# wangjiarui153/AIGV-Assessor

Hardware: AMD Instinct MI355X
Metric: scored clips/sec (8-frame 448x448, InternVL2-8B stage-2 score eval) (higher is better)
Workload: dtype bf16

## Files before the change

### aigv-assessor_amd/csrc/slowfast.hip

```cpp
#include <hip/hip_runtime.h>

#include <algorithm>
#include <cmath>
#include <cstdarg>
#include <cstdio>
#include <cstring>
#include <map>
#include <string>
#include <vector>

#include "../../include/aigv_amd.h"
#include "common.h"
#include "kernels.h"

namespace {

struct ConvArgs {
  const bf16_t* in;
  const bf16_t* w;
  const float* bias;
  const bf16_t* res;
  bf16_t* out;
  int ld_in, Cin, Ti, Hi, Wi;
  int kt, kh, kw, st, sh, sw, pt, ph, pw;
  int To, Ho, Wo, Cout, CoutPad, Kp;
  int ld_res, ld_out, c_off, relu;
  long rows;
  float* part;
  int k_slices;
};

template <int BN>
__global__ __launch_bounds__(256) void conv3d_mfma_kernel(ConvArgs p) {
  constexpr int BM = 128, BK = 64, NT = BN / 16, WJ = (BN + 31) / 32;
  __shared__ __attribute__((aligned(16))) bf16_t sA[BM * BK];
  __shared__ __attribute__((aligned(16))) bf16_t sW[BN * BK];
  const int tid = threadIdx.x, lane = tid & 63, wave = tid >> 6;
  const long m0 = (long)blockIdx.x * BM;
  const int n0 = blockIdx.y * BN;
  const int kspan = p.Kp / p.k_slices, kb = blockIdx.z * kspan;
  const int kc = tid & 7;
  const int r0 = tid >> 3;
  long base[4];
  int t0[4], y0[4], x0[4];
  bool rv[4];
#pragma unroll
  for (int j = 0; j < 4; ++j) {
    const long m = m0 + r0 + 32 * j;
    rv[j] = m < p.rows;
    const long mm = rv[j] ? m : 0;
    const int x = (int)(mm % p.Wo);
    const long r1 = mm / p.Wo;
    const int y = (int)(r1 % p.Ho);
    const long r2 = r1 / p.Ho;
    const int t = (int)(r2 % p.To);
    const long b = r2 / p.To;
    t0[j] = t * p.st - p.pt;
    y0[j] = y * p.sh - p.ph;
    x0[j] = x * p.sw - p.pw;
    base[j] = b * p.Ti * p.Hi * p.Wi;
  }
  int c = kb + kc * 8, dx = 0, dy = 0, dt = 0;
  auto normalise = [&]() {
    while (c >= p.Cin) {
      c -= p.Cin;
      if (++dx == p.kw) {
        dx = 0;
        if (++dy == p.kh) { dy = 0; ++dt; }
      }
    }
  };
  normalise();
  auto gather = [&](int j) -> u16x8 {
    u16x8 z = {0, 0, 0, 0, 0, 0, 0, 0};
    if (!rv[j] || dt >= p.kt) return z;
    const int tt = t0[j] + dt, yy = y0[j] + dy, xx = x0[j] + dx;
    if ((unsigned)tt >= (unsigned)p.Ti || (unsigned)yy >= (unsigned)p.Hi || (unsigned)xx >= (unsigned)p.Wi) return z;
    return *(const u16x8*)(p.in + (base[j] + ((long)tt * p.Hi + yy) * p.Wi + xx) * p.ld_in + c);
  };
  bool wv[WJ];
  const bf16_t* wsrc[WJ];
#pragma unroll
  for (int j = 0; j < WJ; ++j) {
    const int wrow = r0 + 32 * j;
    wv[j] = wrow < BN && (n0 + wrow) < p.CoutPad;
    wsrc[j] = p.w + (size_t)(n0 + (wv[j] ? wrow : 0)) * p.Kp + kb + kc * 8;
  }
  f32x4 acc[2][NT];
#pragma unroll
  for (int i = 0; i < 2; ++i)
#pragma unroll
    for (int n = 0; n < NT; ++n) acc[i][n] = f32x4{0.f, 0.f, 0.f, 0.f};

  const u16x8 zero = {0, 0, 0, 0, 0, 0, 0, 0};
  u16x8 ra[4], rw[WJ];
#pragma unroll
  for (int j = 0; j < 4; ++j) ra[j] = gather(j);
#pragma unroll
  for (int j = 0; j < WJ; ++j) rw[j] = wv[j] ? *(const u16x8*)wsrc[j] : zero;
  const int slot = (kc ^ (r0 & 7)) * 8;
  for (int k0 = 0; k0 < kspan; k0 += BK) {
    __syncthreads();
#pragma unroll
    for (int j = 0; j < 4; ++j) *(u16x8*)&sA[(r0 + 32 * j) * BK + slot] = ra[j];
#pragma unroll
    for (int j = 0; j < WJ; ++j)
      if (r0 + 32 * j < BN) *(u16x8*)&sW[(r0 + 32 * j) * BK + slot] = rw[j];
    __syncthreads();
    if (k0 + BK < kspan) {
      c += BK;
      normalise();
#pragma unroll
      for (int j = 0; j < 4; ++j) ra[j] = gather(j);
#pragma unroll
      for (int j = 0; j < WJ; ++j) rw[j] = wv[j] ? *(const u16x8*)(wsrc[j] + k0 + BK) : zero;
    }
#pragma unroll
    for (int h = 0; h < 2; ++h) {
      const int rs = ((h * 4 + (lane >> 4)) ^ (lane & 7)) * 8;
      bf16x8 a[2], w[NT];
#pragma unroll
      for (int i = 0; i < 2; ++i) a[i] = *(const bf16x8*)&sA[(wave * 32 + i * 16 + (lane & 15)) * BK + rs];
#pragma unroll
      for (int n = 0; n < NT; ++n) w[n] = *(const bf16x8*)&sW[(n * 16 + (lane & 15)) * BK + rs];
#pragma unroll
      for (int i = 0; i < 2; ++i)
#pragma unroll
        for (int n = 0; n < NT; ++n) acc[i][n] = __builtin_amdgcn_mfma_f32_16x16x32_bf16(w[n], a[i], acc[i][n], 0, 0, 0);
    }
  }
#pragma unroll
  for (int i = 0; i < 2; ++i) {
    const long m = m0 + wave * 32 + i * 16 + (lane & 15);
    if (m >= p.rows) continue;
#pragma unroll
    for (int n = 0; n < NT; ++n) {
      const int ch = n0 + n * 16 + (lane >> 4) * 4;
      if (ch >= p.Cout) continue;
      if (p.k_slices > 1) {
        *(f32x4*)(p.part + ((size_t)blockIdx.z * p.rows + m) * p.Cout + ch) = acc[i][n];
        continue;
      }
      float v[4];
#pragma unroll
      for (int e = 0; e < 4; ++e) v[e] = acc[i][n][e] + p.bias[ch + e];
      if (p.res) {
        const u16x4 r = *(const u16x4*)(p.res + m * p.ld_res + ch);
#pragma unroll
        for (int e = 0; e < 4; ++e) v[e] += bf2f(r[e]);
      }
      u16x4 o;
#pragma unroll
      for (int e = 0; e < 4; ++e) o[e] = f2bf(p.relu ? fmaxf(v[e], 0.f) : v[e]);
      *(u16x4*)(p.out + m * p.ld_out + p.c_off + ch) = o;
    }
  }
}

__global__ __launch_bounds__(256) void conv_finalize_kernel(ConvArgs p) {
  const long i = (long)blockIdx.x * 256 + threadIdx.x;
  const int cq = p.Cout >> 2;
  if (i >= p.rows * cq) return;
  const long m = i / cq;
  const int ch = (int)(i - m * cq) * 4;
  f32x4 v = *(const f32x4*)(p.part + (size_t)m * p.Cout + ch);
  for (int z = 1; z < p.k_slices; ++z) v += *(const f32x4*)(p.part + ((size_t)z * p.rows + m) * p.Cout + ch);
#pragma unroll
  for (int e = 0; e < 4; ++e) v[e] += p.bias[ch + e];
  if (p.res) {
    const u16x4 r = *(const u16x4*)(p.res + m * p.ld_res + ch);
#pragma unroll
    for (int e = 0; e < 4; ++e) v[e] += bf2f(r[e]);
  }
  u16x4 o;
#pragma unroll
  for (int e = 0; e < 4; ++e) o[e] = f2bf(p.relu ? fmaxf(v[e], 0.f) : v[e]);
  *(u16x4*)(p.out + m * p.ld_out + p.c_off + ch) = o;
}

struct FrameIdx { int v[64]; };
__global__ __launch_bounds__(256) void sf_repack_kernel(const bf16_t* __restrict__ frames, int T, int Ts, long hw, bf16_t* __restrict__ fast,
                                                        bf16_t* __restrict__ slow, FrameIdx idx, long total) {
  const long i = (long)blockIdx.x * 256 + threadIdx.x;
  if (i >= total) return;
  const long px = i % hw;
  const long f = i / hw;
  const int tt = (int)(f % (T + Ts));
  const long b = f / (T + Ts);
  const int src_t = tt < T ? tt : idx.v[tt - T];
  const bf16_t* s = frames + ((b * T + src_t) * 3) * hw + px;
  u16x4 o = {s[0], s[hw], s[2 * hw], 0};
  bf16_t* d = tt < T ? fast + ((b * T + tt) * hw + px) * 4 : slow + ((b * Ts + (tt - T)) * hw + px) * 4;
  *(u16x4*)d = o;
}

__global__ __launch_bounds__(256) void sf_maxpool_kernel(const bf16_t* __restrict__ in, int C, int Hi, int Wi, int Ho, int Wo,
                                                         bf16_t* __restrict__ out, int ld_out, long total) {
  const long i = (long)blockIdx.x * 256 + threadIdx.x;
  if (i >= total) return;
  const int cv = C >> 3;
  const int c8 = (int)(i % cv);
  const long px = i / cv;
  const int x = (int)(px % Wo);
  const long r = px / Wo;
  const int y = (int)(r % Ho);
  const long f = r / Ho;
  float m[8];
#pragma unroll
  for (int e = 0; e < 8; ++e) m[e] = -INFINITY;
  for (int dy = 0; dy < 3; ++dy) {
    const int yy = 2 * y - 1 + dy;
    if ((unsigned)yy >= (unsigned)Hi) continue;
    for (int dx = 0; dx < 3; ++dx) {
      const int xx = 2 * x - 1 + dx;
      if ((unsigned)xx >= (unsigned)Wi) continue;
      const u16x8 v = *(const u16x8*)(in + ((f * Hi + yy) * Wi + xx) * C + c8 * 8);
#pragma unroll
      for (int e = 0; e < 8; ++e) m[e] = fmaxf(m[e], bf2f(v[e]));
    }
  }
  u16x8 o;
#pragma unroll
  for (int e = 0; e < 8; ++e) o[e] = f2bf(m[e]);
  *(u16x8*)(out + px * ld_out + c8 * 8) = o;
}

struct PoolW { float t[32], y[32], x[32]; };
__global__ __launch_bounds__(256) void sf_pool_kernel(const bf16_t* __restrict__ in, int T, int H, int W, int C, PoolW w,
                                                      bf16_t* __restrict__ out, int ld_out, int c_off) {
  __shared__ float red[64][4][8];
  const int chunk = threadIdx.x & 3, slice = threadIdx.x >> 2;
  const int c8 = blockIdx.x * 4 + chunk;
  const int b = blockIdx.y;
  float acc[8] = {0.f, 0.f, 0.f, 0.f, 0.f, 0.f, 0.f, 0.f};
  if (c8 * 8 < C) {
    const bf16_t* s = in + (long)b * T * H * W * C + c8 * 8;
    const int n = T * H * W;
    for (int i = slice; i < n; i += 64) {
      const int x = i % W, r = i / W, y = r % H, t = r / H;
      const float wt = w.t[t] * w.y[y] * w.x[x];
      const u16x8 v = *(const u16x8*)(s + (long)i * C);
#pragma unroll
      for (int e = 0; e < 8; ++e) acc[e] += wt * bf2f(v[e]);
    }
  }
#pragma unroll
  for (int e = 0; e < 8; ++e) red[slice][chunk][e] = acc[e];
  __syncthreads();
  if (threadIdx.x < 32 && (blockIdx.x * 4 + (threadIdx.x >> 3)) * 8 < C) {
    const int ch = threadIdx.x >> 3, e = threadIdx.x & 7;
    float v = 0.f;
    for (int q = 0; q < 64; ++q) v += red[q][ch][e];
    out[(long)b * ld_out + c_off + (blockIdx.x * 4 + ch) * 8 + e] = f2bf(v);
  }
}

constexpr long SPLITK_MAX_ROWS = 8192;

int conv_k_slices(long rows, int CoutPad, int Kp) {
  if (rows > SPLITK_MAX_ROWS || Kp < 1024) return 1;
  const int bn = CoutPad >= 64 ? 64 : CoutPad >= 32 ? 32 : 16;
  const long tiles = ((rows + 127) / 128) * ((CoutPad + bn - 1) / bn);
  if (tiles >= 64) return 1;
  const int steps = Kp / 64;
  for (int S : {8, 6, 4, 3, 2})
    if (steps % S == 0 && steps / S >= 4 && tiles * S <= 512) return S;
  return 1;
}

hipError_t launch_conv(const ConvArgs& a_in, hipStream_t s, int S = 1, float* ws = nullptr, size_t ws_floats = 0) {
  ConvArgs a = a_in;
  if (a.rows <= 0) return hipSuccess;
  if (a.Cin % 8 || a.ld_in % 8 || a.Cout % 4 || a.ld_out % 4 || a.c_off % 4 || a.Kp % 64 || a.CoutPad % 16 || (a.res && a.ld_res % 4) ||
      a.Kp < a.kt * a.kh * a.kw * a.Cin)
    return hipErrorInvalidValue;
  if (!ws || S < 1 || (a.Kp / 64) % S || (size_t)S * a.rows * a.Cout > ws_floats) S = 1;
  a.k_slices = S;
  a.part = S > 1 ? ws : nullptr;
  const unsigned gx = (unsigned)((a.rows + 127) / 128);
  if (a.CoutPad >= 64) hipLaunchKernelGGL(conv3d_mfma_kernel<64>, dim3(gx, (a.CoutPad + 63) / 64, S), dim3(256), 0, s, a);
  else if (a.CoutPad >= 32) hipLaunchKernelGGL(conv3d_mfma_kernel<32>, dim3(gx, (a.CoutPad + 31) / 32, S), dim3(256), 0, s, a);
  else hipLaunchKernelGGL(conv3d_mfma_kernel<16>, dim3(gx, 1, S), dim3(256), 0, s, a);
  if (S > 1) {
    const long total = a.rows * (a.Cout / 4);
    hipLaunchKernelGGL(conv_finalize_kernel, dim3((unsigned)((total + 255) / 256)), dim3(256), 0, s, a);
  }
  return hipGetLastError();
}

inline uint16_t bf16_host(float f) {
  uint32_t u;
  memcpy(&u, &f, 4);
  if ((u & 0x7fffffffu) > 0x7f800000u) return (uint16_t)((u >> 16) | 0x40);
  u += 0x7fffu + ((u >> 16) & 1u);
  return (uint16_t)(u >> 16);
}
inline float bf16_to_float_host(uint16_t h) {
  uint32_t u = (uint32_t)h << 16;
  float f;
  memcpy(&f, &u, 4);
  return f;
}

struct HostTensor {
  std::vector<float> v;
  std::vector<int64_t> shape;
};

enum OpKind { OP_REPACK, OP_CONV, OP_MAXPOOL, OP_POOL };
struct Op {
  OpKind kind;
  ConvArgs a{};
  int in_buf = -1, out_buf = -1, res_buf = -1;
  size_t w_off = 0, b_off = 0;
  long rows_per_clip = 0;
  int k_slices = 1;
  int C = 0, T = 0, Hi = 0, Wi = 0, Ho = 0, Wo = 0, ld_out = 0, c_off = 0;
  PoolW pw{};
};

int sf_fail(int code, const char* fmt, ...) {
  char buf[768];
  va_list ap;
  va_start(ap, fmt);
  vsnprintf(buf, sizeof buf, fmt, ap);
  va_end(ap);
  aigv_set_error(buf);
  return code;
}

}

struct aigv_slowfast {
  int device = 0, Bcap = 0, T = 0, Ts = 0, H = 0, W = 0;
  bool finalized = false;
  std::map<std::string, HostTensor> host;
  std::vector<Op> ops;
  std::vector<size_t> buf_elems;
  std::vector<bf16_t*> bufs;
  bf16_t* d_w = nullptr;
  float* d_b = nullptr;
  float* d_part = nullptr;
  size_t part_floats = 0;
  FrameIdx slow_idx{};
  double flops_per_clip = 0;
};

namespace {

enum { B_IN0 = 0, B_IN1, B_STEM0, B_STEM1, B_X00, B_X01, B_X10, B_X11, B_A0, B_A1, B_B0, B_B1, B_S0, B_S1, B_COUNT };

struct Builder {
  aigv_slowfast* sf;
  std::vector<uint16_t> w;
  std::vector<float> b;
  std::string missing;

  const HostTensor* get(const std::string& name) {
    auto it = sf->host.find(name);
    if (it == sf->host.end()) {
      if (missing.size() < 400) missing += (missing.empty() ? "" : ", ") + name;
      return nullptr;
    }
    return &it->second;
  }
  void need(int buf, size_t elems) {
    if (sf->buf_elems[buf] < elems) sf->buf_elems[buf] = elems;
  }
  bool conv(const std::string& conv_name, const std::string& norm_name, int in_buf, int ld_in, int cin_eff, int Ti, int Hi, int Wi, int kt, int kh,
            int kw, int st, int sh, int sw, int pt, int ph, int pw, int cout, int out_buf, int ld_out, int c_off, int res_buf, int ld_res, bool relu,
            int* To_, int* Ho_, int* Wo_, bool stem_pairs = false) {
    const HostTensor* W = get(conv_name + ".weight");
    const HostTensor* g = get(norm_name + ".weight");
    const HostTensor* be = get(norm_name + ".bias");
    const HostTensor* mu = get(norm_name + ".running_mean");
    const HostTensor* var = get(norm_name + ".running_var");
    const int To = (Ti + 2 * pt - kt) / st + 1, Ho = (Hi + 2 * ph - kh) / sh + 1, Wo = (Wi + 2 * pw - kw) / sw + 1;
    *To_ = To; *Ho_ = Ho; *Wo_ = Wo;
    if (!W || !g || !be || !mu || !var) return false;
    const int cin_real = W->shape.size() == 5 ? (int)W->shape[1] : -1;
    if (W->shape.size() != 5 || W->shape[0] != cout || (stem_pairs ? cin_real != 3 : cin_real != cin_eff) || W->shape[2] != kt || W->shape[3] != kh || W->shape[4] != kw ||
        (int)g->v.size() != cout || (int)be->v.size() != cout || (int)mu->v.size() != cout || (int)var->v.size() != cout) {
      if (missing.size() < 400) missing += (missing.empty() ? "" : ", ") + conv_name + " (bad shape)";
      return false;
    }
    const int taps = kt * kh * kw;
    const int kw_k = stem_pairs ? 4 : kw, taps_k = kt * kh * kw_k;
    const int K = taps_k * cin_eff, Kp = (K + 63) / 64 * 64, coutPad = (cout + 15) / 16 * 16;
    Op op;
    op.kind = OP_CONV;
    op.w_off = w.size();
    op.b_off = b.size();
    w.resize(w.size() + (size_t)coutPad * Kp, 0);
    b.resize(b.size() + cout, 0.f);
    for (int co = 0; co < cout; ++co) {
      const float scale = g->v[co] / std::sqrt(var->v[co] + 1e-5f);
      b[op.b_off + co] = be->v[co] - mu->v[co] * scale;
      uint16_t* dst = &w[op.w_off + (size_t)co * Kp];
      for (int ci = 0; ci < cin_real; ++ci)
        for (int tap = 0; tap < taps; ++tap) {
          int k = tap * cin_eff + ci;
          if (stem_pairs) {
            const int q = tap % kw + 1;
            k = ((tap / kw) * 4 + (q >> 1)) * 8 + (q & 1) * 4 + ci;
          }
          dst[k] = bf16_host(W->v[((size_t)co * cin_real + ci) * taps + tap] * scale);
        }
    }
    ConvArgs& a = op.a;
    a.ld_in = ld_in; a.Cin = cin_eff; a.Ti = Ti; a.Hi = Hi; a.Wi = stem_pairs ? Wi / 2 : Wi;
    a.kt = kt; a.kh = kh; a.kw = kw_k; a.st = st; a.sh = sh; a.sw = stem_pairs ? 1 : sw; a.pt = pt; a.ph = ph; a.pw = stem_pairs ? 2 : pw;
    a.To = To; a.Ho = Ho; a.Wo = Wo; a.Cout = cout; a.CoutPad = coutPad; a.Kp = Kp;
    a.ld_res = ld_res; a.ld_out = ld_out; a.c_off = c_off; a.relu = relu ? 1 : 0;
    op.in_buf = in_buf; op.out_buf = out_buf; op.res_buf = res_buf;
    op.rows_per_clip = (long)To * Ho * Wo;
    need(out_buf, (size_t)op.rows_per_clip * ld_out);
    sf->flops_per_clip += 2.0 * op.rows_per_clip * cout * (double)taps * cin_real;
    sf->ops.push_back(op);
    return true;
  }
};

void cover_weights(float* w, int n, int k) {
  for (int i = 0; i < n; ++i) {
    const int lo = i - k + 1 > 0 ? i - k + 1 : 0, hi = i < n - k ? i : n - k;
    w[i] = (float)(hi - lo + 1);
  }
}

}

extern "C" {

int aigv_slowfast_create(int device, int max_clips, int frames_per_clip, int height, int width, aigv_slowfast** out) {
  if (!out) return sf_fail(AIGV_ERR_ARG, "aigv_slowfast_create: null argument");
  *out = nullptr;
  int ndev = 0;
  if (hipGetDeviceCount(&ndev) != hipSuccess || ndev <= 0)
    return sf_fail(AIGV_ERR_HIP, "aigv_slowfast_create: no HIP device is visible (this library has no CPU fallback)");
  if (device < 0 || device >= ndev) return sf_fail(AIGV_ERR_ARG, "aigv_slowfast_create: device %d out of range (%d visible)", device, ndev);
  if (max_clips <= 0 || frames_per_clip < 8 || frames_per_clip > 32 || frames_per_clip % 4 || height < 224 || width < 224 || height % 32 ||
      width % 32 || height > 1024 || width > 1024)
    return sf_fail(AIGV_ERR_ARG, "aigv_slowfast_create: needs 8 <= T <= 32 with T %% 4 == 0 and 224 <= H, W <= 1024 multiples of 32 (got T=%d %dx%d)",
                   frames_per_clip, height, width);
  aigv_slowfast* sf = new (std::nothrow) aigv_slowfast();
  if (!sf) return sf_fail(AIGV_ERR_ALLOC, "out of host memory");
  sf->device = device; sf->Bcap = max_clips; sf->T = frames_per_clip; sf->Ts = frames_per_clip / 4; sf->H = height; sf->W = width;
  const int n = sf->Ts;
  const float step = n > 1 ? (float)(sf->T - 1) / (float)(n - 1) : 0.f;
  for (int i = 0; i < n; ++i) sf->slow_idx.v[i] = i < n / 2 ? (int)(0.f + step * i) : (int)((float)(sf->T - 1) - step * (float)(n - 1 - i));
  *out = sf;
  return 0;
}

void aigv_slowfast_destroy(aigv_slowfast* sf) {
  if (!sf) return;
  hipSetDevice(sf->device);
  hipDeviceSynchronize();
  for (bf16_t* p : sf->bufs) hipFree(p);
  hipFree(sf->d_w);
  hipFree(sf->d_b);
  hipFree(sf->d_part);
  delete sf;
}

int aigv_slowfast_load_weight(aigv_slowfast* sf, const char* name, const void* host_data, const int64_t* shape, int ndim, int dtype) {
  if (!sf || !name || !host_data || !shape || ndim <= 0 || ndim > 5) return sf_fail(AIGV_ERR_ARG, "aigv_slowfast_load_weight: bad argument");
  if (sf->finalized) return sf_fail(AIGV_ERR_STATE, "aigv_slowfast_load_weight(%s): already finalized", name);
  std::string key(name);
  for (const char* pre : {"slowfast_model.feature_extraction.", "feature_extraction.", "blocks."}) {
    const size_t n = strlen(pre);
    if (key.compare(0, n, pre) == 0) { key = key.substr(n); break; }
  }
  HostTensor t;
  size_t n = 1;
  for (int i = 0; i < ndim; ++i) {
    if (shape[i] <= 0) return sf_fail(AIGV_ERR_ARG, "aigv_slowfast_load_weight(%s): bad shape", name);
    n *= (size_t)shape[i];
    t.shape.push_back(shape[i]);
  }
  t.v.resize(n);
  if (dtype == AIGV_F32) memcpy(t.v.data(), host_data, n * 4);
  else if (dtype == AIGV_BF16) for (size_t i = 0; i < n; ++i) t.v[i] = bf16_to_float_host(((const uint16_t*)host_data)[i]);
  else return sf_fail(AIGV_ERR_ARG, "aigv_slowfast_load_weight(%s): dtype %d", name, dtype);
  sf->host[key] = std::move(t);
  return 0;
}

int aigv_slowfast_finalize(aigv_slowfast* sf) {
  if (!sf) return sf_fail(AIGV_ERR_ARG, "aigv_slowfast_finalize: null handle");
  if (sf->finalized) return 0;
  if (hipSetDevice(sf->device) != hipSuccess) return sf_fail(AIGV_ERR_HIP, "hipSetDevice failed");
  sf->ops.clear();
  sf->buf_elems.assign(B_COUNT, 0);
  sf->flops_per_clip = 0;
  Builder bd{sf, {}, {}, {}};
  const int T[2] = {sf->Ts, sf->T};
  const int IN[2] = {B_IN0, B_IN1}, STEM[2] = {B_STEM0, B_STEM1}, X[2][2] = {{B_X00, B_X01}, {B_X10, B_X11}}, A[2] = {B_A0, B_A1},
            Bq[2] = {B_B0, B_B1}, S[2] = {B_S0, B_S1};
  {
    Op op; op.kind = OP_REPACK;
    sf->ops.push_back(op);
    bd.need(B_IN0, (size_t)sf->Ts * sf->H * sf->W * 4);
    bd.need(B_IN1, (size_t)sf->T * sf->H * sf->W * 4);
  }
  bool ok = true;
  int h = 0, w = 0, to = 0;
  int ld[2] = {64 + 16, 8};
  for (int p = 0; p < 2; ++p) {
    const int kt = p ? 5 : 1, cout = p ? 8 : 64;
    const std::string pre = "0.multipathway_blocks." + std::to_string(p);
    ok &= bd.conv(pre + ".conv", pre + ".norm", IN[p], 8, 8, T[p], sf->H, sf->W, kt, 7, 7, 1, 2, 2, kt / 2, 3, 3, cout, STEM[p], cout, 0, -1, 0, true, &to, &h, &w, true);
    Op mp; mp.kind = OP_MAXPOOL;
    mp.in_buf = STEM[p]; mp.out_buf = X[p][0]; mp.C = cout; mp.T = T[p]; mp.Hi = h; mp.Wi = w;
    mp.Ho = (h + 2 - 3) / 2 + 1; mp.Wo = (w + 2 - 3) / 2 + 1; mp.ld_out = ld[p];
    bd.need(X[p][0], (size_t)T[p] * mp.Ho * mp.Wo * ld[p]);
    sf->ops.push_back(mp);
    if (p == 1) { h = mp.Ho; w = mp.Wo; }
  }
  int sp_h = h, sp_w = w;
  ok &= bd.conv("0.multipathway_fusion.conv_fast_to_slow", "0.multipathway_fusion.norm", X[1][0], 8, 8, T[1], sp_h, sp_w, 7, 1, 1, 4, 1, 1, 3, 0, 0, 16,
                X[0][0], ld[0], 64, -1, 0, true, &to, &h, &w);
  if (to != T[0]) return sf_fail(AIGV_ERR_ARG, "fast->slow fusion yields %d frames, slow pathway has %d", to, T[0]);
  int cur[2] = {0, 0};
  int cin[2] = {80, 8};
  static const int depths[4] = {3, 4, 6, 3};
  for (int s = 0; s < 4; ++s) {
    int out_h = sp_h, out_w = sp_w;
    for (int p = 0; p < 2; ++p) {
      const int inner = (p ? 8 : 64) << s, cout = inner * 4;
      const int fuse_ch = (s < 3 && p == 0) ? 2 * (32 << s) : 0;
      const int ld_out = cout + fuse_ch;
      const int kt_a = (p == 1 || s >= 2) ? 3 : 1;
      int bh = sp_h, bw = sp_w;
      for (int blk = 0; blk < depths[s]; ++blk) {
        const int stv = (blk == 0 && s > 0) ? 2 : 1;
        const std::string pre = std::to_string(s + 1) + ".multipathway_blocks." + std::to_string(p) + ".res_blocks." + std::to_string(blk) + ".";
        const int xin = X[p][cur[p]], xout = X[p][cur[p] ^ 1];
        const int c_in = blk == 0 ? cin[p] : cout, ld_in = blk == 0 ? ld[p] : ld_out;
        int t1, h1, w1, h2, w2;
        int res_buf = xin, res_ld = ld_in;
        if (blk == 0) {
          ok &= bd.conv(pre + "branch1_conv", pre + "branch1_norm", xin, ld_in, c_in, T[p], bh, bw, 1, 1, 1, 1, stv, stv, 0, 0, 0, cout, S[p], cout, 0, -1, 0,
                        false, &t1, &h1, &w1);
          res_buf = S[p]; res_ld = cout;
        }
        ok &= bd.conv(pre + "branch2.conv_a", pre + "branch2.norm_a", xin, ld_in, c_in, T[p], bh, bw, kt_a, 1, 1, 1, 1, 1, kt_a / 2, 0, 0, inner, A[p], inner, 0,
                      -1, 0, true, &t1, &h1, &w1);
        ok &= bd.conv(pre + "branch2.conv_b", pre + "branch2.norm_b", A[p], inner, inner, T[p], bh, bw, 1, 3, 3, 1, stv, stv, 0, 1, 1, inner, Bq[p], inner, 0, -1,
                      0, true, &t1, &h2, &w2);
        ok &= bd.conv(pre + "branch2.conv_c", pre + "branch2.norm_c", Bq[p], inner, inner, T[p], h2, w2, 1, 1, 1, 1, 1, 1, 0, 0, 0, cout, xout, ld_out, 0, res_buf,
                      res_ld, true, &t1, &h1, &w1);
        bh = h2; bw = w2;
        cur[p] ^= 1;
      }
      cin[p] = ld_out; ld[p] = ld_out;
      out_h = bh; out_w = bw;
    }
    sp_h = out_h; sp_w = out_w;
    if (s < 3) {
      const int cf = 32 << s, cs = 256 << s;
      const std::string pre = std::to_string(s + 1) + ".multipathway_fusion";
      ok &= bd.conv(pre + ".conv_fast_to_slow", pre + ".norm", X[1][cur[1]], cf, cf, T[1], sp_h, sp_w, 7, 1, 1, 4, 1, 1, 3, 0, 0, 2 * cf, X[0][cur[0]], ld[0], cs,
                    -1, 0, true, &to, &h, &w);
    }
  }
  if (!ok) return sf_fail(AIGV_ERR_STATE, "aigv_slowfast_finalize: missing or mis-shaped tensors: %s%s", bd.missing.c_str(), bd.missing.size() >= 400 ? " ..." : "");
  if (sp_h < 7 || sp_w < 7 || sp_h > 32 || sp_w > 32) return sf_fail(AIGV_ERR_ARG, "final map %dx%d outside the head pool's range", sp_h, sp_w);
  for (int p = 0; p < 2; ++p) {
    Op op; op.kind = OP_POOL;
    op.in_buf = X[p][cur[p]]; op.C = p ? 256 : 2048; op.T = T[p]; op.Hi = sp_h; op.Wi = sp_w; op.ld_out = 2304; op.c_off = p ? 2048 : 0;
    const int L = 4 * T[p], k = p ? 32 : 8;
    if (L < k) return sf_fail(AIGV_ERR_ARG, "too few frames for the head pool");
    float rep[128];
    cover_weights(rep, L, k);
    float ty[32], tx[32];
    cover_weights(ty, sp_h, 7);
    cover_weights(tx, sp_w, 7);
    const float nt = (float)(L - k + 1) * k, ny = (float)(sp_h - 6) * 7, nx = (float)(sp_w - 6) * 7;
    for (int t = 0; t < T[p]; ++t) op.pw.t[t] = (rep[4 * t] + rep[4 * t + 1] + rep[4 * t + 2] + rep[4 * t + 3]) / nt;
    for (int y = 0; y < sp_h; ++y) op.pw.y[y] = ty[y] / ny;
    for (int x = 0; x < sp_w; ++x) op.pw.x[x] = tx[x] / nx;
    sf->ops.push_back(op);
  }
  auto dmalloc = [&](void** p, size_t bytes) { return hipMalloc(p, bytes ? bytes : 16); };
  if (dmalloc((void**)&sf->d_w, bd.w.size() * 2) != hipSuccess || dmalloc((void**)&sf->d_b, bd.b.size() * 4) != hipSuccess)
    return sf_fail(AIGV_ERR_ALLOC, "aigv_slowfast_finalize: hipMalloc of %zu weight bytes failed", bd.w.size() * 2);
  if (hipMemcpy(sf->d_w, bd.w.data(), bd.w.size() * 2, hipMemcpyHostToDevice) != hipSuccess ||
      hipMemcpy(sf->d_b, bd.b.data(), bd.b.size() * 4, hipMemcpyHostToDevice) != hipSuccess)
    return sf_fail(AIGV_ERR_HIP, "aigv_slowfast_finalize: weight upload failed");
  sf->bufs.assign(B_COUNT, nullptr);
  for (int i = 0; i < B_COUNT; ++i) {
    const size_t bytes = sf->buf_elems[i] * (size_t)sf->Bcap * 2 + 64;
    if (hipMalloc((void**)&sf->bufs[i], bytes) != hipSuccess) return sf_fail(AIGV_ERR_ALLOC, "aigv_slowfast_finalize: hipMalloc(%zu) failed", bytes);
    if (hipMemset(sf->bufs[i], 0, bytes) != hipSuccess) return sf_fail(AIGV_ERR_HIP, "hipMemset failed");
  }
  size_t need = 0;
  for (Op& op : sf->ops) {
    if (op.kind != OP_CONV) continue;
    op.k_slices = conv_k_slices(op.rows_per_clip, op.a.CoutPad, op.a.Kp);
    if (op.k_slices > 1) need = std::max(need, (size_t)op.k_slices * op.rows_per_clip * sf->Bcap * op.a.Cout);
  }
  sf->part_floats = need;
  if (sf->part_floats && hipMalloc((void**)&sf->d_part, sf->part_floats * sizeof(float)) != hipSuccess)
    return sf_fail(AIGV_ERR_ALLOC, "aigv_slowfast_finalize: hipMalloc of the split-K workspace failed");
  sf->host.clear();
  sf->finalized = true;
  return 0;
}

double aigv_slowfast_flops_per_clip(const aigv_slowfast* sf) { return sf ? sf->flops_per_clip : 0.0; }

int aigv_slowfast_forward(aigv_slowfast* sf, const void* frames_nchw_bf16, int clips, void* feature_bf16, void* stream) {
  if (!sf || !frames_nchw_bf16 || !feature_bf16) return sf_fail(AIGV_ERR_ARG, "aigv_slowfast_forward: null argument");
  if (!sf->finalized) return sf_fail(AIGV_ERR_STATE, "aigv_slowfast_forward: call aigv_slowfast_finalize first");
  if (clips <= 0 || clips > sf->Bcap) return sf_fail(AIGV_ERR_ARG, "aigv_slowfast_forward: %d clips, capacity %d", clips, sf->Bcap);
  if (hipSetDevice(sf->device) != hipSuccess) return sf_fail(AIGV_ERR_HIP, "aigv_slowfast_forward: hipSetDevice(%d) failed", sf->device);
  hipStream_t s = (hipStream_t)stream;
  for (const Op& op : sf->ops) {
    hipError_t e = hipSuccess;
    switch (op.kind) {
      case OP_REPACK: {
        const long hw = (long)sf->H * sf->W, total = (long)clips * (sf->T + sf->Ts) * hw;
        hipLaunchKernelGGL(sf_repack_kernel, dim3((unsigned)((total + 255) / 256)), dim3(256), 0, s, (const bf16_t*)frames_nchw_bf16, sf->T, sf->Ts, hw,
                           sf->bufs[B_IN1], sf->bufs[B_IN0], sf->slow_idx, total);
        e = hipGetLastError();
        break;
      }
      case OP_CONV: {
        ConvArgs a = op.a;
        a.in = sf->bufs[op.in_buf]; a.out = sf->bufs[op.out_buf]; a.res = op.res_buf >= 0 ? sf->bufs[op.res_buf] : nullptr;
        a.w = sf->d_w + op.w_off; a.bias = sf->d_b + op.b_off;
        a.rows = op.rows_per_clip * clips;
        e = launch_conv(a, s, op.k_slices, sf->d_part, sf->part_floats);
        break;
      }
      case OP_MAXPOOL: {
        const long total = (long)clips * op.T * op.Ho * op.Wo * (op.C / 8);
        hipLaunchKernelGGL(sf_maxpool_kernel, dim3((unsigned)((total + 255) / 256)), dim3(256), 0, s, sf->bufs[op.in_buf], op.C, op.Hi, op.Wi, op.Ho, op.Wo,
                           sf->bufs[op.out_buf], op.ld_out, total);
        e = hipGetLastError();
        break;
      }
      case OP_POOL: {
        hipLaunchKernelGGL(sf_pool_kernel, dim3((op.C + 31) / 32, clips), dim3(256), 0, s, sf->bufs[op.in_buf], op.T, op.Hi, op.Wi, op.C, op.pw,
                           (bf16_t*)feature_bf16, op.ld_out, op.c_off);
        e = hipGetLastError();
        break;
      }
    }
    if (e != hipSuccess) return sf_fail(e == hipErrorInvalidValue ? AIGV_ERR_ARG : AIGV_ERR_HIP, "aigv_slowfast_forward: launch failed: %s", hipGetErrorString(e));
  }
  return 0;
}

int aigv_op_conv3d(const void* x, int ld_in, int Cin, int B, const int* dims, const void* w_packed, int Kp, const float* bias, int Cout, const void* res,
                   int ld_res, void* out, int ld_out, int c_off, int relu, void* stream) {
  if (!x || !dims || !w_packed || !bias || !out) return sf_fail(AIGV_ERR_ARG, "aigv_op_conv3d: null argument");
  ConvArgs a{};
  a.in = (const bf16_t*)x; a.ld_in = ld_in; a.Cin = Cin; a.Ti = dims[0]; a.Hi = dims[1]; a.Wi = dims[2];
  a.kt = dims[3]; a.kh = dims[4]; a.kw = dims[5]; a.st = dims[6]; a.sh = dims[7]; a.sw = dims[8]; a.pt = dims[9]; a.ph = dims[10]; a.pw = dims[11];
  if (a.kt <= 0 || a.kh <= 0 || a.kw <= 0 || a.st <= 0 || a.sh <= 0 || a.sw <= 0 || a.pt < 0 || a.ph < 0 || a.pw < 0 || B <= 0 || Cin <= 0 || Cout <= 0 ||
      ld_in < Cin || ld_out < c_off + Cout || (res && ld_res < Cout) || a.Ti + 2 * a.pt < a.kt || a.Hi + 2 * a.ph < a.kh || a.Wi + 2 * a.pw < a.kw)
    return sf_fail(AIGV_ERR_ARG, "aigv_op_conv3d: bad geometry");
  a.To = (a.Ti + 2 * a.pt - a.kt) / a.st + 1; a.Ho = (a.Hi + 2 * a.ph - a.kh) / a.sh + 1; a.Wo = (a.Wi + 2 * a.pw - a.kw) / a.sw + 1;
  a.w = (const bf16_t*)w_packed; a.Kp = Kp; a.bias = bias; a.Cout = Cout; a.CoutPad = (Cout + 15) / 16 * 16;
  a.res = (const bf16_t*)res; a.ld_res = ld_res; a.out = (bf16_t*)out; a.ld_out = ld_out; a.c_off = c_off; a.relu = relu;
  a.rows = (long)B * a.To * a.Ho * a.Wo;
  hipError_t e = launch_conv(a, (hipStream_t)stream);
  if (e != hipSuccess)
    return sf_fail(e == hipErrorInvalidValue ? AIGV_ERR_ARG : AIGV_ERR_HIP,
                   "aigv_op_conv3d (Cin=%d Cout=%d Kp=%d; needs Cin, ld_in %% 8 == 0, Cout, ld_out, c_off %% 4 == 0, Kp %% 64 == 0): %s", Cin, Cout, Kp, hipGetErrorString(e));
  return 0;
}

}
```

Baseline: 34.95.

## Add multi-stage LDS ring pipeline for SlowFast conv3d with direct global-to-LDS loads

Adds a new conv3d kernel that streams A and W tiles into a 2–4 stage shared-memory ring using direct global-to-LDS loads, with explicit vmcnt waits and a single barrier per k-step. The goal is to overlap the implicit-GEMM gathers with MFMA work instead of relying on register double-buffering. A heuristic picks the ring depth from grid size and the LDS budget, falling back to the old kernel otherwise. The epilogue is factored out and preloads bias and residual before the stores, the split-K finalize unrolls its slice loads, and waves_per_eu hints are added. Larger dynamic LDS can reduce occupancy, and the hand-written waitcnt logic is fragile.

```diff
diff --git a/aigv-assessor_amd/csrc/slowfast.hip b/aigv-assessor_amd/csrc/slowfast.hip
--- a/aigv-assessor_amd/csrc/slowfast.hip
+++ b/aigv-assessor_amd/csrc/slowfast.hip
@@ -31,7 +31,59 @@
 };
 
 template <int BN>
-__global__ __launch_bounds__(256) void conv3d_mfma_kernel(ConvArgs p) {
+__device__ __forceinline__ void conv_epilogue(const ConvArgs& p, const f32x4 (&acc)[2][BN / 16], long m0, int n0, int wave, int lane) {
+  constexpr int NT = BN / 16;
+  const long mr[2] = {m0 + wave * 32 + (lane & 15), m0 + wave * 32 + 16 + (lane & 15)};
+  const int ch0 = n0 + (lane >> 4) * 4;
+  if (p.k_slices > 1) {
+#pragma unroll
+    for (int i = 0; i < 2; ++i)
+#pragma unroll
+      for (int n = 0; n < NT; ++n)
+        if (mr[i] < p.rows && ch0 + n * 16 < p.Cout) *(f32x4*)(p.part + ((size_t)blockIdx.z * p.rows + mr[i]) * p.Cout + ch0 + n * 16) = acc[i][n];
+    return;
+  }
+  const long mc[2] = {mr[0] < p.rows ? mr[0] : p.rows - 1, mr[1] < p.rows ? mr[1] : p.rows - 1};
+  float bias[NT][4];
+  u16x4 res[2][NT];
+#pragma unroll
+  for (int n = 0; n < NT; ++n) {
+    const int cc = ch0 + n * 16 < p.Cout ? ch0 + n * 16 : p.Cout - 4;
+#pragma unroll
+    for (int e = 0; e < 4; ++e) bias[n][e] = p.bias[cc + e];
+  }
+  if (p.res) {
+#pragma unroll
+    for (int n = 0; n < NT; ++n) {
+      const int cc = ch0 + n * 16 < p.Cout ? ch0 + n * 16 : p.Cout - 4;
+#pragma unroll
+      for (int i = 0; i < 2; ++i) res[i][n] = *(const u16x4*)(p.res + mc[i] * p.ld_res + cc);
+    }
+  }
+#pragma unroll
+  for (int i = 0; i < 2; ++i) {
+    if (mr[i] >= p.rows) continue;
+#pragma unroll
+    for (int n = 0; n < NT; ++n) {
+      const int ch = ch0 + n * 16;
+      if (ch >= p.Cout) continue;
+      float v[4];
+#pragma unroll
+      for (int e = 0; e < 4; ++e) v[e] = acc[i][n][e] + bias[n][e];
+      if (p.res) {
+#pragma unroll
+        for (int e = 0; e < 4; ++e) v[e] += bf2f(res[i][n][e]);
+      }
+      u16x4 o;
+#pragma unroll
+      for (int e = 0; e < 4; ++e) o[e] = f2bf(p.relu ? fmaxf(v[e], 0.f) : v[e]);
+      *(u16x4*)(p.out + mr[i] * p.ld_out + p.c_off + ch) = o;
+    }
+  }
+}
+
+template <int BN>
+__global__ __launch_bounds__(256) __attribute__((amdgpu_waves_per_eu(4))) void conv3d_mfma_kernel(ConvArgs p) {
   constexpr int BM = 128, BK = 64, NT = BN / 16, WJ = (BN + 31) / 32;
   __shared__ __attribute__((aligned(16))) bf16_t sA[BM * BK];
   __shared__ __attribute__((aligned(16))) bf16_t sW[BN * BK];
@@ -129,33 +181,112 @@
         for (int n = 0; n < NT; ++n) acc[i][n] = __builtin_amdgcn_mfma_f32_16x16x32_bf16(w[n], a[i], acc[i][n], 0, 0, 0);
     }
   }
-#pragma unroll
-  for (int i = 0; i < 2; ++i) {
-    const long m = m0 + wave * 32 + i * 16 + (lane & 15);
-    if (m >= p.rows) continue;
-#pragma unroll
-    for (int n = 0; n < NT; ++n) {
-      const int ch = n0 + n * 16 + (lane >> 4) * 4;
-      if (ch >= p.Cout) continue;
-      if (p.k_slices > 1) {
-        *(f32x4*)(p.part + ((size_t)blockIdx.z * p.rows + m) * p.Cout + ch) = acc[i][n];
-        continue;
+  conv_epilogue<BN>(p, acc, m0, n0, wave, lane);
+}
+
+__device__ __attribute__((aligned(16))) bf16_t g_sf_zero[8];
+
+template <int N>
+__device__ __forceinline__ void wait_vmcnt() { asm volatile("s_waitcnt vmcnt(%0)" ::"n"(N) : "memory"); }
+
+template <int BN, int NS>
+__global__ __launch_bounds__(256) __attribute__((amdgpu_waves_per_eu(4))) void conv3d_ring_kernel(ConvArgs p) {
+  constexpr int BM = 128, BK = 64, NT = BN / 16, WR = BN < 32 ? 32 : BN, WI = WR / 32;
+  constexpr int A_BYTES = BM * BK * 2, STAGE = A_BYTES + WR * BK * 2, NI = 4 + WI;
+  static_assert(NS >= 2 && (NS - 2) * NI <= 63, "vmcnt range");
+  extern __shared__ __attribute__((aligned(16))) char smem[];
+  const int tid = threadIdx.x, lane = tid & 63, wave = tid >> 6;
+  const long m0 = (long)blockIdx.x * BM;
+  const int n0 = blockIdx.y * BN;
+  const int kspan = p.Kp / p.k_slices, kb = blockIdx.z * kspan, steps = kspan / BK;
+  const int r0 = wave * 8 + (lane >> 3);
+  const int kc = (lane & 7) ^ ((lane >> 3) & 7);
+  const bf16_t* const zero = g_sf_zero;
+  long base[4];
+  int t0[4], y0[4], x0[4];
+  bool rv[4];
+#pragma unroll
+  for (int j = 0; j < 4; ++j) {
+    const long m = m0 + r0 + 32 * j;
+    rv[j] = m < p.rows;
+    const long mm = rv[j] ? m : 0;
+    const int x = (int)(mm % p.Wo);
+    const long r1 = mm / p.Wo;
+    const int y = (int)(r1 % p.Ho);
+    const long r2 = r1 / p.Ho;
+    const int t = (int)(r2 % p.To);
+    const long b = r2 / p.To;
+    t0[j] = t * p.st - p.pt;
+    y0[j] = y * p.sh - p.ph;
+    x0[j] = x * p.sw - p.pw;
+    base[j] = b * p.Ti * p.Hi * p.Wi;
+  }
+  int c = kb + kc * 8, dx = 0, dy = 0, dt = 0;
+  auto normalise = [&]() {
+    while (c >= p.Cin) {
+      c -= p.Cin;
+      if (++dx == p.kw) {
+        dx = 0;
+        if (++dy == p.kh) { dy = 0; ++dt; }
       }
-      float v[4];
-#pragma unroll
-      for (int e = 0; e < 4; ++e) v[e] = acc[i][n][e] + p.bias[ch + e];
-      if (p.res) {
-        const u16x4 r = *(const u16x4*)(p.res + m * p.ld_res + ch);
-#pragma unroll
-        for (int e = 0; e < 4; ++e) v[e] += bf2f(r[e]);
-      }
-      u16x4 o;
-#pragma unroll
-      for (int e = 0; e < 4; ++e) o[e] = f2bf(p.relu ? fmaxf(v[e], 0.f) : v[e]);
-      *(u16x4*)(p.out + m * p.ld_out + p.c_off + ch) = o;
-    }
-  }
-}
+    }
+  };
+  normalise();
+  auto gather = [&](int j) -> const bf16_t* {
+    if (!rv[j] || dt >= p.kt) return zero;
+    const int tt = t0[j] + dt, yy = y0[j] + dy, xx = x0[j] + dx;
+    if ((unsigned)tt >= (unsigned)p.Ti || (unsigned)yy >= (unsigned)p.Hi || (unsigned)xx >= (unsigned)p.Wi) return zero;
+    return p.in + (base[j] + ((long)tt * p.Hi + yy) * p.Wi + xx) * p.ld_in + c;
+  };
+  const bf16_t* wsrc[WI];
+#pragma unroll
+  for (int j = 0; j < WI; ++j) {
+    const int wrow = r0 + 32 * j;
+    wsrc[j] = (wrow < BN && n0 + wrow < p.CoutPad) ? p.w + (size_t)(n0 + wrow) * p.Kp + kb + kc * 8 : nullptr;
+  }
+  const unsigned lds0 = __builtin_amdgcn_readfirstlane((unsigned)(size_t)(LDS_AS char*)smem + wave * 1024);
+  auto issue = [&](int k) {
+    if (k >= steps) return;
+    const unsigned dst = lds0 + (unsigned)(k % NS) * STAGE;
+#pragma unroll
+    for (int j = 0; j < 4; ++j) glds16_asm(gather(j), dst + j * 4096);
+#pragma unroll
+    for (int j = 0; j < WI; ++j) glds16_asm(wsrc[j] ? wsrc[j] + k * BK : zero, dst + A_BYTES + j * 4096);
+    c += BK;
+    normalise();
+  };
+  f32x4 acc[2][NT];
+#pragma unroll
+  for (int i = 0; i < 2; ++i)
+#pragma unroll
+    for (int n = 0; n < NT; ++n) acc[i][n] = f32x4{0.f, 0.f, 0.f, 0.f};
+#pragma unroll
+  for (int k = 0; k < NS - 1; ++k) issue(k);
+  for (int k = 0; k < steps; ++k) {
+    if (k + NS - 2 < steps) wait_vmcnt<(NS - 2) * NI>();
+    else wait_vmcnt<0>();
+    asm volatile("s_barrier" ::: "memory");
+    issue(k + NS - 1);
+    const bf16_t* sA = (const bf16_t*)(smem + (k % NS) * STAGE);
+    const bf16_t* sW = (const bf16_t*)(smem + (k % NS) * STAGE + A_BYTES);
+#pragma unroll
+    for (int h = 0; h < 2; ++h) {
+      const int rs = ((h * 4 + (lane >> 4)) ^ (lane & 7)) * 8;
+      bf16x8 a[2], w[NT];
+#pragma unroll
+      for (int i = 0; i < 2; ++i) a[i] = *(const bf16x8*)&sA[(wave * 32 + i * 16 + (lane & 15)) * BK + rs];
+#pragma unroll
+      for (int n = 0; n < NT; ++n) w[n] = *(const bf16x8*)&sW[(n * 16 + (lane & 15)) * BK + rs];
+#pragma unroll
+      for (int i = 0; i < 2; ++i)
+#pragma unroll
+        for (int n = 0; n < NT; ++n) acc[i][n] = __builtin_amdgcn_mfma_f32_16x16x32_bf16(w[n], a[i], acc[i][n], 0, 0, 0);
+    }
+  }
+  conv_epilogue<BN>(p, acc, m0, n0, wave, lane);
+}
+
+constexpr int SPLITK_MAX_SLICES = 8;
 
 __global__ __launch_bounds__(256) void conv_finalize_kernel(ConvArgs p) {
   const long i = (long)blockIdx.x * 256 + threadIdx.x;
@@ -163,8 +294,14 @@
   if (i >= p.rows * cq) return;
   const long m = i / cq;
   const int ch = (int)(i - m * cq) * 4;
-  f32x4 v = *(const f32x4*)(p.part + (size_t)m * p.Cout + ch);
-  for (int z = 1; z < p.k_slices; ++z) v += *(const f32x4*)(p.part + ((size_t)z * p.rows + m) * p.Cout + ch);
+  f32x4 slab[SPLITK_MAX_SLICES];
+#pragma unroll
+  for (int z = 0; z < SPLITK_MAX_SLICES; ++z)
+    slab[z] = *(const f32x4*)(p.part + ((size_t)(z < p.k_slices ? z : p.k_slices - 1) * p.rows + m) * p.Cout + ch);
+  f32x4 v = slab[0];
+#pragma unroll
+  for (int z = 1; z < SPLITK_MAX_SLICES; ++z)
+    if (z < p.k_slices) v += slab[z];
 #pragma unroll
   for (int e = 0; e < 4; ++e) v[e] += p.bias[ch + e];
   if (p.res) {
@@ -268,19 +405,57 @@
   return 1;
 }
 
+#ifndef SF_RING_NS
+#define SF_RING_NS -1
+#endif
+
+int conv_ring_depth(long wgs, int steps, int bn) {
+  if (SF_RING_NS >= 0) return SF_RING_NS;
+  if (steps < 2) return 0;
+  const long stage = 128 * 64 * 2 + (bn < 32 ? 32 : bn) * 64 * 2;
+  for (int ns : {4, 3})
+    if (wgs <= 256L * (160 * 1024 / (std::min(ns, steps) * stage))) return ns;
+  return 0;
+}
+
+template <int BN, int NS>
+hipError_t launch_ring(const ConvArgs& a, dim3 grid, hipStream_t s) {
+  constexpr int stage = 128 * 64 * 2 + (BN < 32 ? 32 : BN) * 64 * 2;
+  static LdsAttrOnce lds_attr;
+  if (hipError_t e = lds_attr.ensure((const void*)conv3d_ring_kernel<BN, NS>, NS * stage); e != hipSuccess) return e;
+  const int steps = a.Kp / a.k_slices / 64;
+  hipLaunchKernelGGL((conv3d_ring_kernel<BN, NS>), grid, dim3(256), std::min(NS, steps) * stage, s, a);
+  return hipSuccess;
+}
+
+template <int BN>
+hipError_t launch_conv_bn(const ConvArgs& a, dim3 grid, int ns, hipStream_t s) {
+  switch (ns) {
+    case 2: return launch_ring<BN, 2>(a, grid, s);
+    case 3: return launch_ring<BN, 3>(a, grid, s);
+    case 4: return launch_ring<BN, 4>(a, grid, s);
+    default: hipLaunchKernelGGL(conv3d_mfma_kernel<BN>, grid, dim3(256), 0, s, a); return hipSuccess;
+  }
+}
+
 hipError_t launch_conv(const ConvArgs& a_in, hipStream_t s, int S = 1, float* ws = nullptr, size_t ws_floats = 0) {
   ConvArgs a = a_in;
   if (a.rows <= 0) return hipSuccess;
   if (a.Cin % 8 || a.ld_in % 8 || a.Cout % 4 || a.ld_out % 4 || a.c_off % 4 || a.Kp % 64 || a.CoutPad % 16 || (a.res && a.ld_res % 4) ||
       a.Kp < a.kt * a.kh * a.kw * a.Cin)
     return hipErrorInvalidValue;
-  if (!ws || S < 1 || (a.Kp / 64) % S || (size_t)S * a.rows * a.Cout > ws_floats) S = 1;
+  if (!ws || S < 1 || S > SPLITK_MAX_SLICES || (a.Kp / 64) % S || (size_t)S * a.rows * a.Cout > ws_floats) S = 1;
   a.k_slices = S;
   a.part = S > 1 ? ws : nullptr;
   const unsigned gx = (unsigned)((a.rows + 127) / 128);
-  if (a.CoutPad >= 64) hipLaunchKernelGGL(conv3d_mfma_kernel<64>, dim3(gx, (a.CoutPad + 63) / 64, S), dim3(256), 0, s, a);
-  else if (a.CoutPad >= 32) hipLaunchKernelGGL(conv3d_mfma_kernel<32>, dim3(gx, (a.CoutPad + 31) / 32, S), dim3(256), 0, s, a);
-  else hipLaunchKernelGGL(conv3d_mfma_kernel<16>, dim3(gx, 1, S), dim3(256), 0, s, a);
+  const int bn = a.CoutPad >= 64 ? 64 : a.CoutPad >= 32 ? 32 : 16;
+  const dim3 grid(gx, (a.CoutPad + bn - 1) / bn, S);
+  const int ns = conv_ring_depth((long)grid.x * grid.y * grid.z, a.Kp / S / 64, bn);
+  hipError_t e = hipSuccess;
+  if (bn == 64) e = launch_conv_bn<64>(a, grid, ns, s);
+  else if (bn == 32) e = launch_conv_bn<32>(a, grid, ns, s);
+  else e = launch_conv_bn<16>(a, grid, ns, s);
+  if (e != hipSuccess) return e;
   if (S > 1) {
     const long total = a.rows * (a.Cout / 4);
     hipLaunchKernelGGL(conv_finalize_kernel, dim3((unsigned)((total + 255) / 256)), dim3(256), 0, s, a);
```

Measured after the change: 34.94 (median of 6 runs). Within noise of the previous version (-0.0%).
